# Go2Heart/StreamFormer

Measured on AMD Instinct MI355X. Metric: frames/s (16x224^2 clips), higher is better.
Workload: dtype bf16; 1 GPU; SigLIP-base StreamFormer encoder forward, 8 clips x 16 x 224^2 per GPU, random-init de-trivialised weights, causal temporal attention; global_batch_clips=8, frames_per_clip=16, parallelism=dp1, steps_in_flight=1

## Files before the change

streamformer_amd/csrc/sf_gemm.hip:

```cpp
#include "sf_common.h"
#include "sf_switches.h"
#include <cstdlib>

#define BM 128
#define BN 128
#define NTHREADS 256

typedef const __attribute__((address_space(1))) void* gptr_t;
typedef __attribute__((address_space(3))) void* lptr_t;

template <int BK>
SF_DEVICE int swz(int row) {
  if (BK == 64) return (row >> 1) & 7;
  return sf_swz64(row);
}

template <int BK>
SF_DEVICE void stage_tile(const bf16_t* __restrict__ X, int row0, int rows_total, int K, int k0,
                          char* lds, int tid) {
  constexpr int CPR = BK / 8;
  constexpr int ROUNDS = BM * CPR / NTHREADS;
  const int wave = tid >> 6;
#pragma unroll
  for (int r = 0; r < ROUNDS; ++r) {
    const int c = r * NTHREADS + tid;
    const int row = c / CPR;
    const int slot = c % CPR;
    const int kc = slot ^ swz<BK>(row);
    int grow = row0 + row;
    grow = grow < rows_total ? grow : rows_total - 1;
    const bf16_t* src = X + (size_t)grow * K + k0 + kc * 8;
    char* dst = lds + (r * NTHREADS + wave * 64) * 16;
    __builtin_amdgcn_global_load_lds((gptr_t)src, (lptr_t)dst, 16, 0, 0);
  }
}

template <int BK>
SF_DEVICE bf16x8_t read_frag(const char* tile, int row, int kc) {
  constexpr int RB = BK * 2;
  const int off = row * RB + ((kc ^ swz<BK>(row)) << 4);
  return *reinterpret_cast<const bf16x8_t*>(tile + off);
}

SF_DEVICE f32x4_t mfma16(bf16x8_t a, bf16x8_t b, f32x4_t c) {
  typedef __attribute__((ext_vector_type(8))) __bf16 v8bf;
  return __builtin_amdgcn_mfma_f32_16x16x32_bf16(__builtin_bit_cast(v8bf, a), __builtin_bit_cast(v8bf, b), c, 0, 0, 0);
}

template <bool SPLIT, int EPI>
__global__ __launch_bounds__(NTHREADS) void sf_gemm_kernel(SfGemmArgs p) {
  constexpr int BK = SPLIT ? 32 : 64;
  constexpr int TILE_BYTES = BM * BK * 2;
  constexpr int STAGE_BYTES = TILE_BYTES * (SPLIT ? 4 : 2);
  extern __shared__ __attribute__((aligned(16))) char smem[];

  const int tid = threadIdx.x;
  const int lane = tid & 63;
  const int wave = tid >> 6;
  const int wr = wave >> 1, wc = wave & 1;
  const int l15 = lane & 15, g = lane >> 4;

  const int tiles_n = (p.N + BN - 1) / BN;
  const int nwg = gridDim.x;
  int bid = blockIdx.x;
  {
    const int xcd = bid & 7, idx = bid >> 3;
    const int q = nwg >> 3, r = nwg & 7;
    bid = (xcd < r ? xcd * (q + 1) : r * (q + 1) + (xcd - r) * q) + idx;
  }
  const int tile_m = bid / tiles_n, tile_n = bid % tiles_n;
  const int m0 = tile_m * BM, n0 = tile_n * BN;

  f32x4_t acc[4][4];
#pragma unroll
  for (int i = 0; i < 4; ++i)
#pragma unroll
    for (int j = 0; j < 4; ++j) acc[i][j] = (f32x4_t){0.f, 0.f, 0.f, 0.f};

  const int nkt = p.K / BK;
  auto stage = [&](int buf, int kt) {
    char* base = smem + buf * STAGE_BYTES;
    stage_tile<BK>(p.a_hi, m0, p.M, p.K, kt * BK, base, tid);
    if (SPLIT) {
      stage_tile<BK>(p.a_lo, m0, p.M, p.K, kt * BK, base + TILE_BYTES, tid);
      stage_tile<BK>(p.w_hi, n0, p.N, p.K, kt * BK, base + 2 * TILE_BYTES, tid);
      stage_tile<BK>(p.w_lo, n0, p.N, p.K, kt * BK, base + 3 * TILE_BYTES, tid);
    } else {
      stage_tile<BK>(p.w_hi, n0, p.N, p.K, kt * BK, base + TILE_BYTES, tid);
    }
  };

  stage(0, 0);
  __syncthreads();

  for (int kt = 0; kt < nkt; ++kt) {
    const int cur = kt & 1;
    if (kt + 1 < nkt) stage(cur ^ 1, kt + 1);
    const char* base = smem + cur * STAGE_BYTES;
    const char* tA = base;
    const char* tAl = base + TILE_BYTES;
    const char* tW = base + (SPLIT ? 2 : 1) * TILE_BYTES;
    const char* tWl = base + 3 * TILE_BYTES;
#pragma unroll
    for (int ks = 0; ks < BK / 32; ++ks) {
      const int kc = ks * 4 + g;
      bf16x8_t xa[4], wa[4];
#pragma unroll
      for (int i = 0; i < 4; ++i) {
        xa[i] = read_frag<BK>(tA, wr * 64 + i * 16 + l15, kc);
        wa[i] = read_frag<BK>(tW, wc * 64 + i * 16 + l15, kc);
      }
      if (SPLIT) {
        bf16x8_t xl[4], wl[4];
#pragma unroll
        for (int i = 0; i < 4; ++i) {
          xl[i] = read_frag<BK>(tAl, wr * 64 + i * 16 + l15, kc);
          wl[i] = read_frag<BK>(tWl, wc * 64 + i * 16 + l15, kc);
        }
#pragma unroll
        for (int nt = 0; nt < 4; ++nt)
#pragma unroll
          for (int mt = 0; mt < 4; ++mt) {
            acc[nt][mt] = mfma16(wl[nt], xa[mt], acc[nt][mt]);
            acc[nt][mt] = mfma16(wa[nt], xl[mt], acc[nt][mt]);
            acc[nt][mt] = mfma16(wa[nt], xa[mt], acc[nt][mt]);
          }
      } else {
#pragma unroll
        for (int nt = 0; nt < 4; ++nt)
#pragma unroll
          for (int mt = 0; mt < 4; ++mt) acc[nt][mt] = mfma16(wa[nt], xa[mt], acc[nt][mt]);
      }
    }
    __syncthreads();
  }

#pragma unroll
  for (int mt = 0; mt < 4; ++mt) {
    const int m = m0 + wr * 64 + mt * 16 + l15;
    if (m >= p.M) continue;
    size_t orow = (size_t)m;
    if (p.grp_rows > 0) orow = sf_out_row(p, m);
#pragma unroll
    for (int nt = 0; nt < 4; ++nt) {
      const int n = n0 + wc * 64 + nt * 16 + g * 4;
      if (n >= p.N) continue;
      f32x4_t v = acc[nt][mt];
      if (p.bias) {
        const f32x4_t b = *reinterpret_cast<const f32x4_t*>(p.bias + n);
        v += b;
      }
      const size_t o = orow * (size_t)p.ldc + n;
      if (EPI == SF_EPI_F32) {
        *reinterpret_cast<f32x4_t*>(p.out_f32 + o) = v;
      } else if (EPI == SF_EPI_RESID_F32) {
        const f32x4_t r = *reinterpret_cast<const f32x4_t*>(p.resid + o);
        v = r + p.alpha * v;
        *reinterpret_cast<f32x4_t*>(p.out_f32 + o) = v;
      } else if (EPI == SF_EPI_EMBED_F32) {
        const int pn = m % p.Np, tt = (m / p.Np) % p.Tn;
        const f32x4_t pe = *reinterpret_cast<const f32x4_t*>(p.pos + (size_t)pn * p.N + n);
        const f32x4_t te = *reinterpret_cast<const f32x4_t*>(p.time_rows + (size_t)tt * p.N + n);
        v = v + pe + te;
        *reinterpret_cast<f32x4_t*>(p.out_f32 + o) = v;
      } else {
        if (EPI == SF_EPI_ACT_BF16) {
#pragma unroll
          for (int j = 0; j < 4; ++j) v[j] = SPLIT ? apply_act(v[j], p.act) : apply_act_bf16(v[j], p.act);
        }
        unsigned int h[4], l[4];
#pragma unroll
        for (int j = 0; j < 4; ++j) split_bf(v[j], h[j], l[j]);
        u32x2_t hv = {h[0] | (h[1] << 16), h[2] | (h[3] << 16)};
        *reinterpret_cast<u32x2_t*>(p.out_hi + o) = hv;
        if (p.out_lo) {
          u32x2_t lv = {l[0] | (l[1] << 16), l[2] | (l[3] << 16)};
          *reinterpret_cast<u32x2_t*>(p.out_lo + o) = lv;
        }
      }
    }
  }
}

template <bool SPLIT>
static hipError_t launch_epi(const SfGemmArgs& a, dim3 grid, size_t lds, hipStream_t s) {
#define SF_CASE(E) case E: return sf_launch_big_lds(sf_gemm_kernel<SPLIT, E>, grid, dim3(NTHREADS), lds, s, a);
  switch (a.epi) {
    SF_CASE(SF_EPI_F32)
    SF_CASE(SF_EPI_BF16)
    SF_CASE(SF_EPI_ACT_BF16)
    SF_CASE(SF_EPI_RESID_F32)
    SF_CASE(SF_EPI_EMBED_F32)
    default:
      return hipErrorInvalidValue;
  }
#undef SF_CASE
}

int sf_wall_clock_ticks(int ns) {
  static int khz = 0;
  if (!khz) {
    int dev = 0, rate = 0;
    if (hipGetDevice(&dev) == hipSuccess && hipDeviceGetAttribute(&rate, hipDeviceAttributeWallClockRate, dev) == hipSuccess && rate > 0) khz = rate;
    else khz = 100000;
  }
  return (int)((long long)ns * khz / 1000000);
}

int sf_infold_max_rows() {
  const int a = sf_skinny_max_rows(), b = sf_tile_max_rows();
  return a > b ? a : b;
}

SfGemmFamily sf_gemm_family(const SfGemmArgs& a, bool split) {
  if (a.aux_mode) return sf_gemm256_aux_supported(a) && !split ? SF_GEMM_FAM_G256 : SF_GEMM_FAM_NONE;
  if (a.ln_inkernel) {
    if (sf_gemm_skinny_supported(a, split)) return SF_GEMM_FAM_SKINNY;
    return sf_gemm_tile_supported(a, split) ? SF_GEMM_FAM_TILE : SF_GEMM_FAM_NONE;
  }
  if (sf_gemm_skinny_supported(a, split) && !sf_sw(SW_DISABLE_SKINNY)) return SF_GEMM_FAM_SKINNY;
  if (sf_gemm_tile_supported(a, split)) return SF_GEMM_FAM_TILE;
#ifdef SF_LAB
  if (sf_gemm_pipe_supported(a, split)) return SF_GEMM_FAM_LAB_PIPE;
  if (sf_gemm_pp_supported(a, split)) return SF_GEMM_FAM_LAB_PP;
#endif
  if (sf_gemm_panel_supported(a, split)) return SF_GEMM_FAM_PANEL;
  if (sf_gemm256_supported(a, split)) return SF_GEMM_FAM_G256;
  if (a.resid_hi) return SF_GEMM_FAM_NONE;
  if (a.N % 256 == 128 && a.N > 256 && !a.ln_stats && !a.ln_stats_out && a.epi != SF_EPI_EMBED_F32 && !sf_sw(SW_DISABLE_GEMM_COLSPLIT)) {
    SfGemmArgs m = a;
    m.N = a.N - 128;
    if (sf_gemm256_supported(m, split)) return SF_GEMM_FAM_COLSPLIT;
  }
  return SF_GEMM_FAM_G128;
}

hipError_t sf_launch_gemm_family(SfGemmFamily fam, const SfGemmArgs& a, bool split, hipStream_t s) {
  switch (fam) {
    case SF_GEMM_FAM_SKINNY: return sf_launch_gemm_skinny(a, split, s);
    case SF_GEMM_FAM_TILE: return sf_launch_gemm_tile(a, s);
#ifdef SF_LAB
    case SF_GEMM_FAM_LAB_PIPE: return sf_launch_gemm_pipe(a, s);
    case SF_GEMM_FAM_LAB_PP: return sf_launch_gemm_pp(a, s);
#endif
    case SF_GEMM_FAM_PANEL: return sf_launch_gemm_panel(a, s);
    case SF_GEMM_FAM_G256: return sf_launch_gemm256(a, s);
    case SF_GEMM_FAM_COLSPLIT: {
      SfGemmArgs m = a;
      m.N = a.N - 128;
      SfGemmArgs t = a;
      const size_t n0 = (size_t)m.N;
      t.N = 128;
      t.w_hi = a.w_hi + n0 * a.K; if (a.w_lo) t.w_lo = a.w_lo + n0 * a.K;
      if (a.bias) t.bias = a.bias + n0;
      if (a.resid) t.resid = a.resid + n0;
      if (a.out_f32) t.out_f32 = a.out_f32 + n0;
      if (a.out_hi) t.out_hi = a.out_hi + n0;
      if (a.out_lo) t.out_lo = a.out_lo + n0;
      if (a.aux) t.aux = a.aux + n0;
      const hipError_t e = sf_launch_gemm256(m, s);
      if (e != hipSuccess) return e;
      return sf_launch_gemm128(t, split, s);
    }
    case SF_GEMM_FAM_G128: return sf_launch_gemm128(a, split, s);
    default: return hipErrorInvalidValue;
  }
}

hipError_t sf_launch_gemm(const SfGemmArgs& a, bool split, hipStream_t s) { return sf_launch_gemm_family(sf_gemm_family(a, split), a, split, s); }

bool sf_gemm128_supported(const SfGemmArgs& a, bool split) {
  const int bk = split ? 32 : 64;
  if (a.M <= 0 || a.N <= 0 || a.K <= 0 || (a.K % bk) || (a.N % 4) || (a.ldc % 4)) return false;
  if (split && (!a.a_lo || !a.w_lo)) return false;
  if (a.aux_mode || a.ln_stats || a.ln_stats_out || a.ln_inkernel || a.resid_hi || a.resid_mod > 0 || a.out_lo2) return false;
  switch (a.epi) {
    case SF_EPI_F32: return a.out_f32 != nullptr;
    case SF_EPI_RESID_F32: return a.out_f32 && a.resid;
    case SF_EPI_EMBED_F32: return a.out_f32 && a.pos && a.time_rows && a.Np > 0 && a.Tn > 0;
    case SF_EPI_BF16: case SF_EPI_ACT_BF16: return a.out_hi != nullptr;
    default: return false;
  }
}

hipError_t sf_launch_gemm128(const SfGemmArgs& a, bool split, hipStream_t s) {
  const int bk = split ? 32 : 64;
  if (a.M <= 0 || a.N <= 0 || a.K <= 0 || (a.K % bk) || (a.N % 4) || (a.ldc % 4)) return hipErrorInvalidValue;
  if (split && (!a.a_lo || !a.w_lo)) return hipErrorInvalidValue;
  const int tiles = ((a.M + BM - 1) / BM) * ((a.N + BN - 1) / BN);
  const size_t lds = 2 * (size_t)BM * 64 * 2 * 2;
  return split ? launch_epi<true>(a, dim3(tiles), lds, s) : launch_epi<false>(a, dim3(tiles), lds, s);
}
```

streamformer_amd/csrc/sf_gemm_panel.hip:

```cpp
#include "sf_common.h"
#include "sf_switches.h"
#include <cstdlib>

#define P_THREADS 512
#define P_NT 3
#define P_SLOT_BYTES 40960
#define P_A_BYTES 16384

typedef __attribute__((address_space(3))) void* lptr_t;

SF_DEVICE f32x4_t mfma16p(bf16x8_t a, bf16x8_t b, f32x4_t c) {
  typedef __attribute__((ext_vector_type(8))) __bf16 v8bf;
  return __builtin_amdgcn_mfma_f32_16x16x32_bf16(__builtin_bit_cast(v8bf, a), __builtin_bit_cast(v8bf, b), c, 0, 0, 0);
}
template <int N>
SF_DEVICE void wait_vmp() {
  asm volatile("s_waitcnt vmcnt(%0)" ::"n"(N) : "memory");
}
SF_DEVICE bf16x8_t rd32(const char* piece, int row, int kc) {
  return *reinterpret_cast<const bf16x8_t*>(piece + row * 64 + ((kc ^ sf_swz64(row)) << 4));
}

#ifdef SF_PANEL_TRACE
__device__ unsigned long long panel_trace[16];
#define PT_DECL unsigned long long pt_[6] = {0, 0, 0, 0, 0, 0}, pt_t = 0, pt_0 = 0
#define PT_START() do { pt_t = pt_0 = __builtin_amdgcn_s_memtime(); } while (0)
#define PT_MARK(i) do { const unsigned long long pt_n = __builtin_amdgcn_s_memtime(); pt_[i] += pt_n - pt_t; pt_t = pt_n; } while (0)
#define PT_FLUSH() do { if (lane == 0) { for (int i_ = 0; i_ < 6; ++i_) atomicAdd(&panel_trace[i_], pt_[i_]); \
    atomicAdd(&panel_trace[6], __builtin_amdgcn_s_memtime() - pt_0); atomicAdd(&panel_trace[7], 1ull); } } while (0)
#define PT_OFF(bit) ((SF_PANEL_TRACE) & (bit))
#else
#define PT_DECL
#define PT_START()
#define PT_MARK(i)
#define PT_FLUSH()
#define PT_OFF(bit) 0
#endif

template <int P_MT>
__global__ __launch_bounds__(P_THREADS) void sf_gemm_panel_kernel(SfGemmArgs p, int rows_per_tile, int ntiles, int stagger_ticks, int pad_clamp) {
  extern __shared__ __attribute__((aligned(16))) char smem[];
  const int tid = threadIdx.x;
  const int lane = tid & 63;
  const int wave = __builtin_amdgcn_readfirstlane(tid >> 6);
  const int half = wave >> 2;
  const int l15 = lane & 15, g = lane >> 4;
  const int K = p.K;
  const int nkt = K >> 5;
  if (stagger_ticks > 0) {
    const int grp = (blockIdx.x >> 4) % 3;
    if (grp) {
      const unsigned long long t0 = wall_clock64();
      while (wall_clock64() - t0 < (unsigned long long)grp * (unsigned long long)stagger_ticks) __builtin_amdgcn_s_sleep(8);
    }
  }
  for (int bid = blockIdx.x; bid < ntiles; bid += gridDim.x) {
  const int panel = (bid >> 4) * 8 + (bid & 7), nh = (bid >> 3) & 1;
  const int m0 = panel * rows_per_tile;
  const int m_end = min(m0 + rows_per_tile, p.M);
  const int n0 = nh * 384;
  if (m0 >= p.M) continue;

  const __amdgpu_buffer_rsrc_t rsrc_a = __builtin_amdgcn_make_buffer_rsrc((void*)p.a_hi, 0, (unsigned)p.M * (unsigned)K * 2u, 0x00020000);
  const __amdgpu_buffer_rsrc_t rsrc_w = __builtin_amdgcn_make_buffer_rsrc((void*)p.w_hi, 0, (unsigned)p.N * (unsigned)K * 2u, 0x00020000);
  unsigned offA[2], offW[3];
#pragma unroll
  for (int i = 0; i < 3; ++i) {
    const int c = i * P_THREADS + tid;
    const int row = c >> 2, kc = (c & 3) ^ sf_swz64(row);
    if (i < 2) {
      const int ar = m0 + row;
      offA[i] = (ar < m_end || pad_clamp) ? ((unsigned)(ar < m_end ? ar : m_end - 1) * (unsigned)K + kc * 8) * 2u : 0xffff0000u;
    }
    offW[i] = ((unsigned)(n0 + row) * (unsigned)K + kc * 8) * 2u;
  }
  const int dma_lds = wave * 1024;
  auto issue = [&](int t) {
    char* dst = smem + (t & 3) * P_SLOT_BYTES + dma_lds;
    const int kof = t * 64;
    __builtin_amdgcn_raw_ptr_buffer_load_lds(rsrc_a, (lptr_t)dst, 16, offA[0], kof, 0, 0);
    __builtin_amdgcn_raw_ptr_buffer_load_lds(rsrc_a, (lptr_t)(dst + 8192), 16, offA[1], kof, 0, 0);
    __builtin_amdgcn_raw_ptr_buffer_load_lds(rsrc_w, (lptr_t)(dst + P_A_BYTES), 16, offW[0], kof, 0, 0);
    __builtin_amdgcn_raw_ptr_buffer_load_lds(rsrc_w, (lptr_t)(dst + P_A_BYTES + 8192), 16, offW[1], kof, 0, 0);
    __builtin_amdgcn_raw_ptr_buffer_load_lds(rsrc_w, (lptr_t)(dst + P_A_BYTES + 16384), 16, offW[2], kof, 0, 0);
  };

  PT_DECL;
  PT_START();
  f32x4_t acc[P_MT][P_NT];
#pragma unroll
  for (int i = 0; i < P_MT; ++i)
#pragma unroll
    for (int j = 0; j < P_NT; ++j) acc[i][j] = (f32x4_t){0.f, 0.f, 0.f, 0.f};
  bf16x8_t af[P_MT], wf[P_NT];

  auto reads = [&](int t) {
    const char* pa = smem + (t & 3) * P_SLOT_BYTES;
    const char* pw = pa + P_A_BYTES;
#pragma unroll
    for (int nt = 0; nt < P_NT; ++nt) wf[nt] = rd32(pw, wave * 48 + nt * 16 + l15, g);
#pragma unroll
    for (int mt = 0; mt < P_MT; ++mt) af[mt] = rd32(pa, mt * 16 + l15, g);
  };
  auto mma = [&]() {
    __builtin_amdgcn_s_setprio(1);
#pragma unroll
    for (int mt = 0; mt < P_MT; ++mt)
#pragma unroll
      for (int nt = 0; nt < P_NT; ++nt) acc[mt][nt] = mfma16p(wf[nt], af[mt], acc[mt][nt]);
    __builtin_amdgcn_s_setprio(0);
  };

  int t = 0;
  if (half == 1) {
    issue(0); issue(1); issue(2);
    wait_vmp<10>();
    __builtin_amdgcn_s_barrier();
    __builtin_amdgcn_s_barrier();
    for (; t + 3 < nkt; ++t) {
      issue(t + 3);
      reads(t);
      wait_vmp<10>();
      __builtin_amdgcn_s_barrier();
      mma();
      __builtin_amdgcn_s_barrier();
    }
    reads(t); wait_vmp<5>(); __builtin_amdgcn_s_barrier(); mma(); __builtin_amdgcn_s_barrier(); ++t;
    reads(t); wait_vmp<0>(); __builtin_amdgcn_s_barrier(); mma(); __builtin_amdgcn_s_barrier(); ++t;
    reads(t); __builtin_amdgcn_s_barrier(); mma(); __builtin_amdgcn_s_barrier();
  } else {
    issue(0); issue(1);
    wait_vmp<5>();
    __builtin_amdgcn_s_barrier();
    for (; t + 2 < nkt; ++t) {
      issue(t + 2);
      reads(t);
      wait_vmp<5>();
      __builtin_amdgcn_s_barrier();
      mma();
      __builtin_amdgcn_s_barrier();
    }
    reads(t); wait_vmp<0>(); __builtin_amdgcn_s_barrier(); mma(); __builtin_amdgcn_s_barrier(); ++t;
    reads(t); __builtin_amdgcn_s_barrier(); mma(); __builtin_amdgcn_s_barrier();
    __builtin_amdgcn_s_barrier();
  }

#ifdef SF_LAB
  if (p.w_nt >= 78) {
    const int lm = p.w_nt - 78;
    if (lm == 2 || (lm == 1 && (blockIdx.x & 1)) || (lm == 3 && (blockIdx.x & 3))) {
      if (acc[0][0][0] == 12345.678f) p.out_hi[0] = 0;
      continue;
    }
  }
#endif
  PT_MARK(0);
  int tid_e = threadIdx.x;
  asm volatile("" : "+v"(tid_e));
  const int el15 = tid_e & 15, eg = (tid_e >> 4) & 3;
  f32x4_t bias4[P_NT];
#pragma unroll
  for (int nt = 0; nt < P_NT; ++nt)
    bias4[nt] = p.bias ? *reinterpret_cast<const f32x4_t*>(p.bias + n0 + wave * 48 + nt * 16 + eg * 4)
                       : (f32x4_t){0.f, 0.f, 0.f, 0.f};
  const int elane = tid_e & 63;
#pragma unroll
  for (int grp = 0; grp < (P_MT + 3) / 4; ++grp) {
    constexpr int kRows = 8;
    const int rows_w = (grp + 1) * 4 <= P_MT ? kRows : 2 * (P_MT - grp * 4);
    f32x4_t res[kRows][2];
#pragma unroll
    for (int j = 0; j < kRows; ++j) {
      const int m = m0 + grp * 64 + wave + 8 * j;
      if (p.resid_hi) {
        u32x4_t h = {0u, 0u, 0u, 0u}, l = {0u, 0u, 0u, 0u};
        if (j < rows_w && m < m_end && elane < 48 && !PT_OFF(2)) {
          const size_t ro = (size_t)m * (size_t)p.ldc + n0 + elane * 8;
          h = *reinterpret_cast<const u32x4_t*>(p.resid_hi + ro);
          l = *reinterpret_cast<const u32x4_t*>(p.resid_lo + ro);
        }
        res[j][0] = __builtin_bit_cast(f32x4_t, h);
        res[j][1] = __builtin_bit_cast(f32x4_t, l);
        continue;
      }
      const bool ok = j < rows_w && m < m_end && p.resid != nullptr;
      const int mr = p.resid_mod > 0 ? m % p.resid_mod : m;
      const float* rp = p.resid + (size_t)mr * (size_t)p.ldc + n0;
      res[j][0] = ok ? *reinterpret_cast<const f32x4_t*>(rp + elane * 4) : (f32x4_t){0.f, 0.f, 0.f, 0.f};
      res[j][1] = (ok && elane < 32) ? *reinterpret_cast<const f32x4_t*>(rp + 256 + elane * 4) : (f32x4_t){0.f, 0.f, 0.f, 0.f};
    }
#pragma unroll
    for (int q = 0; q < 4; ++q) {
      const int mt = grp * 4 + q;
      if (mt < P_MT) {
        const int r = q * 16 + el15;
#pragma unroll
        for (int nt = 0; nt < P_NT; ++nt) {
          const int chunk = wave * 12 + nt * 4 + eg;
          const f32x4_t v = acc[mt][nt] + bias4[nt];
          *reinterpret_cast<f32x4_t*>(smem + r * 1536 + (((chunk & ~31) | ((chunk ^ r) & 31)) << 4)) = v;
        }
      }
    }
    PT_MARK(1);
    __syncthreads();
    PT_MARK(2);
#pragma unroll
    for (int j = 0; j < kRows; ++j) {
      const int r = wave + 8 * j;
      const int m = m0 + grp * 64 + r;
      if (j < rows_w && m < m_end) {
        float s1 = 0.f, s2 = 0.f;
        if (p.resid_hi) {
          if (elane < 48) {
            const u32x4_t h = __builtin_bit_cast(u32x4_t, res[j][0]), l = __builtin_bit_cast(u32x4_t, res[j][1]);
            u32x4_t ho, lo;
#pragma unroll
            for (int hf = 0; hf < 2; ++hf) {
              const int c = 2 * elane + hf;
              const f32x4_t v = *reinterpret_cast<const f32x4_t*>(smem + r * 1536 + (((c & ~31) | ((c ^ r) & 31)) << 4));
              f32x4_t x;
              x[0] = bf2f(h[2 * hf] & 0xffffu) + bf2f(l[2 * hf] & 0xffffu) + p.alpha * v[0];
              x[1] = bf2f(h[2 * hf] >> 16) + bf2f(l[2 * hf] >> 16) + p.alpha * v[1];
              x[2] = bf2f(h[2 * hf + 1] & 0xffffu) + bf2f(l[2 * hf + 1] & 0xffffu) + p.alpha * v[2];
              x[3] = bf2f(h[2 * hf + 1] >> 16) + bf2f(l[2 * hf + 1] >> 16) + p.alpha * v[3];
              ho[2 * hf] = pack_bf2(x[0], x[1]); ho[2 * hf + 1] = pack_bf2(x[2], x[3]);
              lo[2 * hf] = pack_bf2(x[0] - bf2f(ho[2 * hf] & 0xffffu), x[1] - bf2f(ho[2 * hf] >> 16));
              lo[2 * hf + 1] = pack_bf2(x[2] - bf2f(ho[2 * hf + 1] & 0xffffu), x[3] - bf2f(ho[2 * hf + 1] >> 16));
              s1 += (x[0] + x[1]) + (x[2] + x[3]);
              s2 += (x[0] * x[0] + x[1] * x[1]) + (x[2] * x[2] + x[3] * x[3]);
            }
            const size_t o = (size_t)m * (size_t)p.ldc + n0 + elane * 8;
            if (!PT_OFF(4) || s1 == 12345.678f) {
              *reinterpret_cast<u32x4_t*>(p.out_hi + o) = ho;
              *reinterpret_cast<u32x4_t*>(p.out_lo + o) = lo;
            }
          }
        } else
#pragma unroll
        for (int hp = 0; hp < 2; ++hp) {
          const int c = hp * 64 + elane;
          if (hp == 0 || elane < 32) {
            const f32x4_t v = *reinterpret_cast<const f32x4_t*>(smem + r * 1536 + (((c & ~31) | ((c ^ r) & 31)) << 4));
            const f32x4_t x = res[j][hp] + p.alpha * v;
            const size_t o = (size_t)m * (size_t)p.ldc + n0 + c * 4;
            if (p.out_f32) *reinterpret_cast<f32x4_t*>(p.out_f32 + o) = x;
            if (p.out_hi) {
              const u32x2_t hv = {pack_bf2(x[0], x[1]), pack_bf2(x[2], x[3])};
              *reinterpret_cast<u32x2_t*>(p.out_hi + o) = hv;
              if (p.out_lo)
                *reinterpret_cast<u32x2_t*>(p.out_lo + o) = (u32x2_t){pack_bf2(x[0] - bf2f(hv[0] & 0xffffu), x[1] - bf2f(hv[0] >> 16)),
                                                                    pack_bf2(x[2] - bf2f(hv[1] & 0xffffu), x[3] - bf2f(hv[1] >> 16))};
              s1 += (x[0] + x[1]) + (x[2] + x[3]);
              s2 += (x[0] * x[0] + x[1] * x[1]) + (x[2] * x[2] + x[3] * x[3]);
            }
          }
        }
        if (p.ln_stats_out) {
          s1 = wave_sum_dpp(s1);
          s2 = wave_sum_dpp(s2);
          if (elane == 0) {
            p.ln_stats_out[(size_t)m * 8 + nh * 4 + 0] = s1;
            p.ln_stats_out[(size_t)m * 8 + nh * 4 + 1] = s2;
          }
        }
      }
    }
    PT_MARK(3);
    __syncthreads();
    PT_MARK(4);
  }
  PT_FLUSH();
  }
}

static int panel_cus() {
  int cus = sf_device_cus();
  if (cus < 16) cus = 256;
  return cus & ~15;
}

struct PanelPlan { int panels, rows, mt, ok; };
static PanelPlan panel_plan(int M) {
  PanelPlan pl = {0, 0, 0, 0};
  const int half = panel_cus() / 2;
  int panels = ((M + 207) / 208 + half - 1) / half * half;
  if (panels <= 0) return pl;
  const int rows = (M + panels - 1) / panels;
  static const int kMt[4] = {2, 4, 7, 13};
  for (int i = 0; i < 4; ++i)
    if (rows <= 16 * kMt[i]) { pl.mt = kMt[i]; break; }
  if (!pl.mt) return pl;
  const int forced = sf_sw(SW_PANEL_MIN_FILL_PCT) ? atoi(sf_sw(SW_PANEL_MIN_FILL_PCT)) : 0;
  const int min_fill = forced ? forced : (M >= 14000 ? 55 : 75);
  pl.panels = panels; pl.rows = rows; pl.ok = rows * 100 >= pl.mt * 16 * min_fill;
  return pl;
}

bool sf_gemm_panel_supported(const SfGemmArgs& a, bool split) {
  if (split || a.N != 768 || a.grp_rows > 0) return false;
  if (a.out_lo && (a.epi != SF_EPI_RESID_F32 || !a.out_hi)) return false;
  if (a.resid_hi && (!a.resid_lo || !a.out_lo || a.epi != SF_EPI_RESID_F32 || a.resid_mod > 0)) return false;
  if (a.epi != SF_EPI_RESID_F32 && a.epi != SF_EPI_F32 && a.epi != SF_EPI_BF16) return false;
  if (a.ln_stats) return false;
  if (a.ln_stats_out && !a.ln_stats_wide) return false;
  if (a.K % 32 || a.K < 128) return false;
  if ((size_t)a.M * a.K * 2 >= ((size_t)1 << 32)) return false;
  return panel_plan(a.M).ok != 0;
}

hipError_t sf_launch_gemm_panel(const SfGemmArgs& a_in, hipStream_t s) {
  SfGemmArgs a = a_in;
  if (a.epi == SF_EPI_F32) { a.resid = nullptr; a.alpha = 1.f; a.out_hi = nullptr; }
  if (a.epi == SF_EPI_BF16) { a.resid = nullptr; a.alpha = 1.f; a.out_f32 = nullptr; }
  const PanelPlan pl = panel_plan(a.M);
  if (!pl.ok) return hipErrorInvalidValue;
  const int cus = panel_cus();
  const int ntiles = pl.panels * 2;
  int stagger = (ntiles >= cus && pl.mt == 13) ? sf_wall_clock_ticks(3500) : 0;
  if (const char* e = sf_sw(SW_PANEL_STAGGER_NS)) stagger = sf_wall_clock_ticks(atoi(e));
  if (const int lm = SF_LAB_SWITCH("SF_PANEL_LAB_EPI")) a.w_nt = 78 + lm;
  const int pad_clamp = sf_sw(SW_PANEL_PAD_CLAMP) ? 1 : 0;
  const dim3 grid(ntiles < cus ? ntiles : cus), block(P_THREADS);
  const size_t lds = 4 * P_SLOT_BYTES;
  switch (pl.mt) {
    case 2: return sf_launch_big_lds(sf_gemm_panel_kernel<2>, grid, block, lds, s, a, pl.rows, ntiles, stagger, pad_clamp);
    case 4: return sf_launch_big_lds(sf_gemm_panel_kernel<4>, grid, block, lds, s, a, pl.rows, ntiles, stagger, pad_clamp);
    case 7: return sf_launch_big_lds(sf_gemm_panel_kernel<7>, grid, block, lds, s, a, pl.rows, ntiles, stagger, pad_clamp);
    default: return sf_launch_big_lds(sf_gemm_panel_kernel<13>, grid, block, lds, s, a, pl.rows, ntiles, stagger, pad_clamp);
  }
}
```

streamformer_amd/csrc/sf_switches.h:

```cpp
#pragma once

#define SF_SWITCH_TABLE(X) \
  X(ACC_TWO_PLANES, "SF_ACC_TWO_PLANES", "accurate mode: residual stream as two planes instead of three (A/B; max-abs 1.4e-4 instead of 5e-5)") \
  X(ASSUME_CUS, "SF_ASSUME_CUS", "size persistent grids for this many CUs (CU-masked stream experiments)") \
  X(DISABLE_ACC_FOLD, "SF_DISABLE_ACC_FOLD", "accurate mode: fp32 residual + standalone LayerNorm instead of the folded plane form (A/B)") \
  X(DISABLE_G256_SPLIT, "SF_DISABLE_G256_SPLIT", "accurate mode: keep the bf16x3 GEMMs off the persistent 256-column kernel") \
  X(DISABLE_GEMM_COLSPLIT, "SF_DISABLE_GEMM_COLSPLIT", "N = 256 j + 128 (so400m widths): the whole GEMM on 128^2 tiles instead of 256-column kernel + a 128-column tail (A/B)") \
  X(DISABLE_GEMM_MID, "SF_DISABLE_GEMM_MID", "skinny family: no 64 x 64 tiles above 512 rows") \
  X(DISABLE_GEMM_TILE, "SF_DISABLE_GEMM_TILE", "one / two clips per call: no tile-GEMM family") \
  X(DISABLE_LN_FOLD, "SF_DISABLE_LN_FOLD", "bf16 mode: standalone LayerNorm launches instead of the fold into the consumer GEMMs (A/B)") \
  X(DISABLE_RESID_PLANES, "SF_DISABLE_RESID_PLANES", "bf16 mode: fp32 residual stream instead of hi + lo planes (A/B)") \
  X(DISABLE_SKG_UNROLL, "SF_DISABLE_SKG_UNROLL", "streaming: K-parallel skinny GEMM with a run-time K-tile count (A/B)") \
  X(DISABLE_SKINNY, "SF_DISABLE_SKINNY", "send small-M GEMMs to the generic 128^2 kernel") \
  X(DISABLE_SPATIAL_DMA, "SF_DISABLE_SPATIAL_DMA", "spatial attention on the register-staged kernel") \
  X(DISABLE_SPATIAL_DMA_ACC, "SF_DISABLE_SPATIAL_DMA_ACC", "accurate mode: spatial attention on fp32 q / k / v (test coverage of that path)") \
  X(DISABLE_SPATIAL_NTC, "SF_DISABLE_SPATIAL_NTC", "spatial attention with a run-time tile count (A/B)") \
  X(DISABLE_STREAM_FOLD, "SF_DISABLE_STREAM_FOLD", "streaming: standalone LayerNorm launches (A/B)") \
  X(DISABLE_STREAM_GRAPH, "SF_DISABLE_STREAM_GRAPH", "streaming: eager launches instead of hipGraph replay") \
  X(DISABLE_TEMPORAL_DECODE, "SF_DISABLE_TEMPORAL_DECODE", "streaming: general temporal kernel instead of the single-query one") \
  X(TBWD_OWN_CU, "SF_TBWD_OWN_CU", "training: temporal attention backward as 12-wave workgroups that own a CU instead of 4-wave workgroups with their exact LDS (bit-identical, 65 against 51 us per launch; for jobs that share a device, DESIGN.md 4)") \
  X(TEMPORAL_DECODE_LANE_KEY, "SF_TEMPORAL_DECODE_LANE_KEY", "streaming: single-query temporal kernel with one key per lane (A/B against whole-line loads)") \
  X(DISABLE_TEMPORAL_DMA, "SF_DISABLE_TEMPORAL_DMA", "temporal attention on the register-staged kernel") \
  X(DISABLE_TEMPORAL_DMA_ACC, "SF_DISABLE_TEMPORAL_DMA_ACC", "accurate mode: temporal attention on fp32 q / k / v (test coverage of that path)") \
  X(EMBED_VIA_GEMM128, "SF_EMBED_VIA_GEMM128", "embedding GEMM on the generic kernel (A/B)") \
  X(G256_FORCE_BM, "SF_G256_FORCE_BM", "256-column kernel: force the row-tile height (tests of the short tiles)") \
  X(G256_NO_BM224, "SF_G256_NO_BM224", "256-column kernel: no 224-row tiles") \
  X(G256_NO_SHORT_BM, "SF_G256_NO_SHORT_BM", "256-column kernel, accurate mode: no 160 / 192-row tiles") \
  X(G256_SPLIT_MIN_N, "SF_G256_SPLIT_MIN_N", "accurate mode: smallest N the persistent kernel takes") \
  X(G256_WALK, "SF_G256_WALK", "256-column kernel: column-group width (tiles) of the column-group-major tile walk, 0 = row-major (A/B of the fabric traffic)") \
  X(G256_STORE_WT, "SF_G256_STORE_WT", "256-column kernel: bf16 outputs leave with write-through (sc1) stores that do not stay in the XCD's L2 (A/B)") \
  X(G256_STORE_NT, "SF_G256_STORE_NT", "256-column kernel: bf16 outputs leave with non-temporal stores (A/B: do the residual planes then survive in the Infinity Cache?)") \
  X(G256_STAGGER_GROUPS, "SF_G256_STAGGER_GROUPS", "256-column kernel: phase-stagger groups per XCD") \
  X(G256_STAGGER_NS, "SF_G256_STAGGER_NS", "256-column kernel: stagger step in ns (overrides the percentage)") \
  X(G256_STAGGER_ONLY, "SF_G256_STAGGER_ONLY", "256-column kernel: stagger only some launches (A/B)") \
  X(G256_STAGGER_PCT, "SF_G256_STAGGER_PCT", "256-column kernel: stagger step as a percentage of the tile period") \
  X(GEMM_MID_MIN_M, "SF_GEMM_MID_MIN_M", "skinny family: first M of the 64 x 64 tiles") \
  X(LN_BWD_BLOCKS, "SF_LN_BWD_BLOCKS", "LayerNorm backward: workgroups (tuning)") \
  X(POOL_SHARE_CU, "SF_POOL_SHARE_CU", "pooling head: the probe / combine kernels request only the LDS they use instead of a CU's whole 160 KB (A/B; with it other workgroups share their CUs, see DESIGN.md 4 on device sharing)") \
  X(PANEL_MIN_FILL_PCT, "SF_PANEL_MIN_FILL_PCT", "panel kernel: minimum last-round fill") \
  X(PANEL_PAD_CLAMP, "SF_PANEL_PAD_CLAMP", "panel kernel: clamp instead of zero-fill the padding rows (A/B)") \
  X(PANEL_STAGGER_NS, "SF_PANEL_STAGGER_NS", "panel kernel: phase-stagger step in ns") \
  X(SKINNY_MAX_M, "SF_SKINNY_MAX_M", "skinny family: largest M") \
  X(SKINNY_NO_KG, "SF_SKINNY_NO_KG", "skinny family: no K-parallel variant") \
  X(SKINNY_NB, "SF_SKINNY_NB", "streaming, folded skinny consumers: 1 = 32 x 32 tiles everywhere, 2 / 3 = force 32 x 64 / 32 x 96 tiles (A/B)") \
  X(SKINNY_NT, "SF_SKINNY_NT", "skinny family: non-temporal weight loads (A/B)") \
  X(SKINNY_TPS, "SF_SKINNY_TPS", "skinny family: tiles per slot (tuning)") \
  X(SPATIAL_PERS, "SF_SPATIAL_PERS", "lab library: persistent spatial attention kernel") \
  X(SPATIAL_TPW, "SF_SPATIAL_TPW", "spatial attention: query tiles per workgroup (tuning)") \
  X(STREAM_GRAPH_PER_POSITION, "SF_STREAM_GRAPH_PER_POSITION", "streaming: one graph per cache position instead of the position-free one (A/B)") \
  X(TILE_FOLD_MIN_M, "SF_TILE_FOLD_MIN_M", "tile-GEMM family: smallest M whose LayerNorm fold uses a statistics buffer and the 256^2 consumers") \
  X(TILE_MAX_M, "SF_TILE_MAX_M", "tile-GEMM family: largest M") \
  X(TILE_MIN_M, "SF_TILE_MIN_M", "tile-GEMM family: smallest M") \
  X(TILE_SHAPE, "SF_TILE_SHAPE", "tile-GEMM family: force a tile shape (tools/tile_lab.py)") \
  X(TRAIN_UNFUSED_TEMPORAL, "SF_TRAIN_UNFUSED_TEMPORAL", "training: temporal_attention.output.dense and temporal_dense as two launches instead of one fused projection (A/B)") \
  X(TRAIN_SIDE_STREAM, "SF_TRAIN_SIDE_STREAM", "training: 0 keeps the LoRA gradients on the caller stream (A/B)") \
  X(WGRAD_NSPLIT, "SF_WGRAD_NSPLIT", "weight-gradient GEMM: force the token splits") \
  X(WGRAD_SMALL_TILES, "SF_WGRAD_SMALL_TILES", "weight-gradient GEMM: 128^2 tiles only") \
  X(WGRAD_UNGROUPED, "SF_WGRAD_UNGROUPED", "training: one weight-gradient launch per projection instead of one per layer (test / A/B)") \

enum SfSw {
#define SF_SW_ENUM(id, name, what) SW_##id,
  SF_SWITCH_TABLE(SF_SW_ENUM)
#undef SF_SW_ENUM
  SW_COUNT
};
const char* sf_sw(SfSw k);
```

Before: 15650 frames/s.

## Skip unused A-row DMA in panel GEMM and use full-height row tiles

The panel GEMM kernel now issues the A-piece buffer-to-LDS loads only for waves whose rows an MFMA actually reads, and the vmcnt waits are adjusted to match the reduced load count. The panel plan switches from M/P evenly split rows to full 16*MT-row tiles with the panel count rounded up to a multiple of 8. The phase stagger now applies to every MT=13 launch. The kernel also gains a K=64 path, but the dispatcher still routes only K>=128 to it. This cuts wasted global traffic and LDS writes for padding rows, at the cost of a changed tile-to-CU distribution that could leave the last round unbalanced.

```diff
diff --git a/streamformer_amd/csrc/sf_gemm.hip b/streamformer_amd/csrc/sf_gemm.hip
--- a/streamformer_amd/csrc/sf_gemm.hip
+++ b/streamformer_amd/csrc/sf_gemm.hip
@@ -224,7 +224,7 @@
   if (sf_gemm_pipe_supported(a, split)) return SF_GEMM_FAM_LAB_PIPE;
   if (sf_gemm_pp_supported(a, split)) return SF_GEMM_FAM_LAB_PP;
 #endif
-  if (sf_gemm_panel_supported(a, split)) return SF_GEMM_FAM_PANEL;
+  if (a.K >= 128 && sf_gemm_panel_supported(a, split)) return SF_GEMM_FAM_PANEL;
   if (sf_gemm256_supported(a, split)) return SF_GEMM_FAM_G256;
   if (a.resid_hi) return SF_GEMM_FAM_NONE;
   if (a.N % 256 == 128 && a.N > 256 && !a.ln_stats && !a.ln_stats_out && a.epi != SF_EPI_EMBED_F32 && !sf_sw(SW_DISABLE_GEMM_COLSPLIT)) {
diff --git a/streamformer_amd/csrc/sf_gemm_panel.hip b/streamformer_amd/csrc/sf_gemm_panel.hip
--- a/streamformer_amd/csrc/sf_gemm_panel.hip
+++ b/streamformer_amd/csrc/sf_gemm_panel.hip
@@ -16,6 +16,12 @@
 template <int N>
 SF_DEVICE void wait_vmp() {
   asm volatile("s_waitcnt vmcnt(%0)" ::"n"(N) : "memory");
+}
+template <int AHEAD>
+SF_DEVICE void wait_refills(int na) {
+  if (na == 2) wait_vmp<5 * AHEAD>();
+  else if (na == 1) wait_vmp<4 * AHEAD>();
+  else wait_vmp<3 * AHEAD>();
 }
 SF_DEVICE bf16x8_t rd32(const char* piece, int row, int kc) {
   return *reinterpret_cast<const bf16x8_t*>(piece + row * 64 + ((kc ^ sf_swz64(row)) << 4));
@@ -38,7 +44,7 @@
 #endif
 
 template <int P_MT>
-__global__ __launch_bounds__(P_THREADS) void sf_gemm_panel_kernel(SfGemmArgs p, int rows_per_tile, int ntiles, int stagger_ticks, int pad_clamp) {
+__global__ __launch_bounds__(P_THREADS) void sf_gemm_panel_kernel(SfGemmArgs p, int rows_per_tile, int ntiles, int stagger_ticks, int pad_clamp, int dma_rows) {
   extern __shared__ __attribute__((aligned(16))) char smem[];
   const int tid = threadIdx.x;
   const int lane = tid & 63;
@@ -75,11 +81,13 @@
     offW[i] = ((unsigned)(n0 + row) * (unsigned)K + kc * 8) * 2u;
   }
   const int dma_lds = wave * 1024;
+  const bool dma_a0 = P_MT > 8 || wave * 16 < dma_rows, dma_a1 = 128 + wave * 16 < dma_rows;
+  const int na = (int)dma_a0 + (int)dma_a1;
   auto issue = [&](int t) {
     char* dst = smem + (t & 3) * P_SLOT_BYTES + dma_lds;
     const int kof = t * 64;
-    __builtin_amdgcn_raw_ptr_buffer_load_lds(rsrc_a, (lptr_t)dst, 16, offA[0], kof, 0, 0);
-    __builtin_amdgcn_raw_ptr_buffer_load_lds(rsrc_a, (lptr_t)(dst + 8192), 16, offA[1], kof, 0, 0);
+    if (dma_a0) __builtin_amdgcn_raw_ptr_buffer_load_lds(rsrc_a, (lptr_t)dst, 16, offA[0], kof, 0, 0);
+    if (dma_a1) __builtin_amdgcn_raw_ptr_buffer_load_lds(rsrc_a, (lptr_t)(dst + 8192), 16, offA[1], kof, 0, 0);
     __builtin_amdgcn_raw_ptr_buffer_load_lds(rsrc_w, (lptr_t)(dst + P_A_BYTES), 16, offW[0], kof, 0, 0);
     __builtin_amdgcn_raw_ptr_buffer_load_lds(rsrc_w, (lptr_t)(dst + P_A_BYTES + 8192), 16, offW[1], kof, 0, 0);
     __builtin_amdgcn_raw_ptr_buffer_load_lds(rsrc_w, (lptr_t)(dst + P_A_BYTES + 16384), 16, offW[2], kof, 0, 0);
@@ -113,29 +121,29 @@
 
   int t = 0;
   if (half == 1) {
-    issue(0); issue(1); issue(2);
-    wait_vmp<10>();
+    issue(0); issue(1);
+    if (nkt > 2) { issue(2); wait_refills<2>(na); } else wait_refills<1>(na);
     __builtin_amdgcn_s_barrier();
     __builtin_amdgcn_s_barrier();
     for (; t + 3 < nkt; ++t) {
       issue(t + 3);
       reads(t);
-      wait_vmp<10>();
+      wait_refills<2>(na);
       __builtin_amdgcn_s_barrier();
       mma();
       __builtin_amdgcn_s_barrier();
     }
-    reads(t); wait_vmp<5>(); __builtin_amdgcn_s_barrier(); mma(); __builtin_amdgcn_s_barrier(); ++t;
+    if (nkt > 2) { reads(t); wait_refills<1>(na); __builtin_amdgcn_s_barrier(); mma(); __builtin_amdgcn_s_barrier(); ++t; }
     reads(t); wait_vmp<0>(); __builtin_amdgcn_s_barrier(); mma(); __builtin_amdgcn_s_barrier(); ++t;
     reads(t); __builtin_amdgcn_s_barrier(); mma(); __builtin_amdgcn_s_barrier();
   } else {
     issue(0); issue(1);
-    wait_vmp<5>();
+    wait_refills<1>(na);
     __builtin_amdgcn_s_barrier();
     for (; t + 2 < nkt; ++t) {
       issue(t + 2);
       reads(t);
-      wait_vmp<5>();
+      wait_refills<1>(na);
       __builtin_amdgcn_s_barrier();
       mma();
       __builtin_amdgcn_s_barrier();
@@ -286,14 +294,23 @@
   const int half = panel_cus() / 2;
   int panels = ((M + 207) / 208 + half - 1) / half * half;
   if (panels <= 0) return pl;
-  const int rows = (M + panels - 1) / panels;
+  int rows = (M + panels - 1) / panels;
   static const int kMt[4] = {2, 4, 7, 13};
   for (int i = 0; i < 4; ++i)
     if (rows <= 16 * kMt[i]) { pl.mt = kMt[i]; break; }
   if (!pl.mt) return pl;
   const int forced = sf_sw(SW_PANEL_MIN_FILL_PCT) ? atoi(sf_sw(SW_PANEL_MIN_FILL_PCT)) : 0;
   const int min_fill = forced ? forced : (M >= 14000 ? 55 : 75);
-  pl.panels = panels; pl.rows = rows; pl.ok = rows * 100 >= pl.mt * 16 * min_fill;
+  pl.ok = rows * 100 >= pl.mt * 16 * min_fill;
+  if (const char* e = sf_sw(SW_PANEL_FORCE_MT)) {
+    const int mt = atoi(e);
+    if ((mt == 2 || mt == 4 || mt == 7 || mt == 13) && mt >= pl.mt) { pl.mt = mt; pl.ok = 1; }
+  }
+  if (!sf_sw(SW_PANEL_EVEN_ROWS)) {
+    rows = 16 * pl.mt;
+    panels = ((M + rows - 1) / rows + 7) & ~7;
+  }
+  pl.panels = panels; pl.rows = rows;
   return pl;
 }
 
@@ -304,7 +321,7 @@
   if (a.epi != SF_EPI_RESID_F32 && a.epi != SF_EPI_F32 && a.epi != SF_EPI_BF16) return false;
   if (a.ln_stats) return false;
   if (a.ln_stats_out && !a.ln_stats_wide) return false;
-  if (a.K % 32 || a.K < 128) return false;
+  if (a.K % 32 || a.K < 64) return false;
   if ((size_t)a.M * a.K * 2 >= ((size_t)1 << 32)) return false;
   return panel_plan(a.M).ok != 0;
 }
@@ -317,16 +334,17 @@
   if (!pl.ok) return hipErrorInvalidValue;
   const int cus = panel_cus();
   const int ntiles = pl.panels * 2;
-  int stagger = (ntiles >= cus && pl.mt == 13) ? sf_wall_clock_ticks(3500) : 0;
+  int stagger = pl.mt == 13 ? sf_wall_clock_ticks(3500) : 0;
   if (const char* e = sf_sw(SW_PANEL_STAGGER_NS)) stagger = sf_wall_clock_ticks(atoi(e));
   if (const int lm = SF_LAB_SWITCH("SF_PANEL_LAB_EPI")) a.w_nt = 78 + lm;
   const int pad_clamp = sf_sw(SW_PANEL_PAD_CLAMP) ? 1 : 0;
+  const int dma_rows = sf_sw(SW_PANEL_DMA_ALL_ROWS) ? 256 : 16 * pl.mt;
   const dim3 grid(ntiles < cus ? ntiles : cus), block(P_THREADS);
   const size_t lds = 4 * P_SLOT_BYTES;
   switch (pl.mt) {
-    case 2: return sf_launch_big_lds(sf_gemm_panel_kernel<2>, grid, block, lds, s, a, pl.rows, ntiles, stagger, pad_clamp);
-    case 4: return sf_launch_big_lds(sf_gemm_panel_kernel<4>, grid, block, lds, s, a, pl.rows, ntiles, stagger, pad_clamp);
-    case 7: return sf_launch_big_lds(sf_gemm_panel_kernel<7>, grid, block, lds, s, a, pl.rows, ntiles, stagger, pad_clamp);
-    default: return sf_launch_big_lds(sf_gemm_panel_kernel<13>, grid, block, lds, s, a, pl.rows, ntiles, stagger, pad_clamp);
-  }
-}
+    case 2: return sf_launch_big_lds(sf_gemm_panel_kernel<2>, grid, block, lds, s, a, pl.rows, ntiles, stagger, pad_clamp, dma_rows);
+    case 4: return sf_launch_big_lds(sf_gemm_panel_kernel<4>, grid, block, lds, s, a, pl.rows, ntiles, stagger, pad_clamp, dma_rows);
+    case 7: return sf_launch_big_lds(sf_gemm_panel_kernel<7>, grid, block, lds, s, a, pl.rows, ntiles, stagger, pad_clamp, dma_rows);
+    default: return sf_launch_big_lds(sf_gemm_panel_kernel<13>, grid, block, lds, s, a, pl.rows, ntiles, stagger, pad_clamp, dma_rows);
+  }
+}
diff --git a/streamformer_amd/csrc/sf_switches.h b/streamformer_amd/csrc/sf_switches.h
--- a/streamformer_amd/csrc/sf_switches.h
+++ b/streamformer_amd/csrc/sf_switches.h
@@ -37,6 +37,9 @@
   X(GEMM_MID_MIN_M, "SF_GEMM_MID_MIN_M", "skinny family: first M of the 64 x 64 tiles") \
   X(LN_BWD_BLOCKS, "SF_LN_BWD_BLOCKS", "LayerNorm backward: workgroups (tuning)") \
   X(POOL_SHARE_CU, "SF_POOL_SHARE_CU", "pooling head: the probe / combine kernels request only the LDS they use instead of a CU's whole 160 KB (A/B; with it other workgroups share their CUs, see DESIGN.md 4 on device sharing)") \
+  X(PANEL_DMA_ALL_ROWS, "SF_PANEL_DMA_ALL_ROWS", "panel kernel: every wave issues both A-piece DMA instructions of a K-tile, also those whose rows no MFMA reads (A/B; bit-identical)") \
+  X(PANEL_EVEN_ROWS, "SF_PANEL_EVEN_ROWS", "panel kernel: M / P rows per tile, P a multiple of half the CUs, instead of full 16 MT-row tiles (A/B; bit-identical)") \
+  X(PANEL_FORCE_MT, "SF_PANEL_FORCE_MT", "panel kernel: force the m-tile count of a row tile (2 / 4 / 7 / 13; tests of every instance at small M)") \
   X(PANEL_MIN_FILL_PCT, "SF_PANEL_MIN_FILL_PCT", "panel kernel: minimum last-round fill") \
   X(PANEL_PAD_CLAMP, "SF_PANEL_PAD_CLAMP", "panel kernel: clamp instead of zero-fill the padding rows (A/B)") \
   X(PANEL_STAGGER_NS, "SF_PANEL_STAGGER_NS", "panel kernel: phase-stagger step in ns") \
```

Measured after the change: 15660 frames/s (median of 4 runs). About the same (+0.1%).
